# COMP6248-Reproducability-Challenge/selfsupervised-denoising

Measured on AMD Instinct MI355X. Metric: training patches/sec (64x64 gauss25 SSDN), higher is better.
Workload: dtype f16

## Files before the change

selfsupervised-denoising_amd/csrc/api.hip:

```cpp
#include "common.h"
#include <cstdarg>
#include <cstdio>
#include <cstdlib>

static thread_local char g_err[512] = "";
thread_local hipEvent_t g_ssdn_stop_event = nullptr;
thread_local bool g_ssdn_stop_used = false;
thread_local hipEvent_t g_ssdn_prof_start = nullptr, g_ssdn_prof_stop = nullptr;
thread_local bool g_ssdn_prof_used = false;

int ssdn_set_error(const char* fmt, ...) {
    va_list ap;
    va_start(ap, fmt);
    vsnprintf(g_err, sizeof(g_err), fmt, ap);
    va_end(ap);
    return -1;
}

#include <vector>
struct ProfSlot {
    bool on = false;
    std::vector<hipEvent_t> ev;
    size_t used = 0;
    double flops = 0.0, bytes = 0.0;
// ... 236 lines not shown
            armed = true;
        };
        switch (ops[i].type) {
            case SSDN_OP_PACK_INPUT: {
                const bool next_conv = i + 1 < n && ops[i + 1].type == SSDN_OP_CONV && ops[i + 1].args && (one_lane ? 0 : ops[i + 1].lane) == lane;
                if (next_conv && chain_merging_on() && conv_pack_fusable((const ssdn_pack_input_args*)p, (const ssdn_conv_args*)ops[i + 1].args)) {
                    rc = launch_conv_thin((const ssdn_conv_args*)ops[i + 1].args, (const ssdn_pack_input_args*)p, s);
                    ++i;
                } else rc = launch_pack_input((const ssdn_pack_input_args*)p, s);
                break;
            }
            case SSDN_OP_CONV: {
                const int m = chain_len(ops + i, n - i, one_lane);
                if (m < 0) return -1;
                const bool pair = m <= 1 && i + 1 < n && ops[i + 1].type == SSDN_OP_CONV && ops[i + 1].args && (one_lane ? 0 : ops[i + 1].lane) == lane &&
                                  chain_merging_on() && conv_pair_fusable((const ssdn_conv_args*)p, (const ssdn_conv_args*)ops[i + 1].args);
                arm(i + (m > 1 ? m : (pair ? 2 : 1)));
                if (m > 1) { rc = launch_chain(ops + i, m, one_lane, s); i += m - 1; }
                else if (pair) { rc = launch_gemm_dma_with_next((const ssdn_conv_args*)p, (const ssdn_conv_args*)ops[i + 1].args, s); ++i; }
                else rc = launch_conv((const ssdn_conv_args*)p, s);
                break;
            }
            case SSDN_OP_POOL_FWD: rc = launch_pool_fwd((const ssdn_pool_args*)p, s); break;
            case SSDN_OP_POOL_BWD: arm(i + 1); rc = launch_pool_bwd((const ssdn_pool_args*)p, s); break;
            case SSDN_OP_UPSUM_BWD: arm(i + 1); rc = launch_upsum_bwd((const ssdn_upsum_args*)p, s); break;
            case SSDN_OP_UNROT_FWD: rc = launch_unrot_fwd((const ssdn_unrot_args*)p, s); break;
            case SSDN_OP_UNROT_BWD: arm(i + 1); rc = launch_unrot_bwd((const ssdn_unrot_args*)p, s); break;
            case SSDN_OP_WGRAD: {
                static const bool no_merge = ssdn_tuning_env("SSDN_NO_WGRAD_MERGE") != nullptr;
                {
                    const ssdn_wgrad_args* mg[WGRAD_MEGA_MAX];
                    int mm = 0;
                    while (!no_merge && mm < WGRAD_MEGA_MAX && i + mm < n && ops[i + mm].type == SSDN_OP_WGRAD && ops[i + mm].args &&
                           (one_lane ? 0 : ops[i + mm].lane) == lane && wgrad_mega_ok((const ssdn_wgrad_args*)ops[i + mm].args) &&
                           ((const ssdn_wgrad_args*)ops[i + mm].args)->mega == ((const ssdn_wgrad_args*)p)->mega)
                        mg[mm] = (const ssdn_wgrad_args*)ops[i + mm].args, ++mm;
                    if (mm > 1) { arm(i + mm); rc = launch_wgrad_mega(mg, mm, s); i += mm - 1; break; }
                }
                const ssdn_wgrad_args* items[WGRAD_MULTI_MAX];
                int m = 0;
                while (!no_merge && m < WGRAD_MULTI_MAX && i + m < n && ops[i + m].type == SSDN_OP_WGRAD && ops[i + m].args &&
                       (one_lane ? 0 : ops[i + m].lane) == lane && wgrad_mergeable((const ssdn_wgrad_args*)ops[i + m].args))
                    items[m] = (const ssdn_wgrad_args*)ops[i + m].args, ++m;
                if (m > 1) { rc = launch_wgrad_multi(items, m, s); i += m - 1; }
                else rc = launch_wgrad((const ssdn_wgrad_args*)p, s);
                break;
            }
            case SSDN_OP_WREDUCE: {
                const ssdn_wreduce_args* items[WREDUCE_MULTI_MAX];
                int m = 0;
                while (m < WREDUCE_MULTI_MAX && i + m < n && ops[i + m].type == SSDN_OP_WREDUCE && ops[i + m].args &&
                       (one_lane ? 0 : ops[i + m].lane) == lane)
                    items[m] = (const ssdn_wreduce_args*)ops[i + m].args, ++m;
                arm_last(i + m);
                rc = m > 1 ? launch_wreduce_multi(items, m, s) : launch_wreduce((const ssdn_wreduce_args*)p, s);
                i += m - 1;
                break;
            }
            case SSDN_OP_WPACK: {
                const ssdn_wpack_args* items[WPACK_MULTI_MAX];
                int m = 0;
                while (m < WPACK_MULTI_MAX && i + m < n && ops[i + m].type == SSDN_OP_WPACK && ops[i + m].args &&
                       (one_lane ? 0 : ops[i + m].lane) == lane)
                    items[m] = (const ssdn_wpack_args*)ops[i + m].args, ++m;
                rc = m > 1 ? launch_wpack_multi(items, m, s) : launch_wpack((const ssdn_wpack_args*)p, s);
                i += m - 1;
                break;
            }
            case SSDN_OP_GRAD_PACK: {
                const bool next_conv = i + 1 < n && ops[i + 1].type == SSDN_OP_CONV && ops[i + 1].args && (one_lane ? 0 : ops[i + 1].lane) == lane;
                if (next_conv && chain_merging_on() && conv_gradpack_fusable((const ssdn_grad_pack_args*)p, (const ssdn_conv_args*)ops[i + 1].args)) {
                    arm(i + 2);
                    rc = launch_gradpack_dgrad((const ssdn_grad_pack_args*)p, (const ssdn_conv_args*)ops[i + 1].args, s);
                    ++i;
                } else { arm(i + 1); rc = launch_grad_pack((const ssdn_grad_pack_args*)p, s); }
                break;
            }
            case SSDN_OP_HEAD_SSDN: rc = launch_head((const ssdn_head_args*)p, s); break;
            case SSDN_OP_HEAD_FINAL: rc = launch_head_final((const ssdn_head_final_args*)p, s); break;
            case SSDN_OP_SPATIAL_MEAN: rc = launch_spatial_mean((const ssdn_spatial_mean_args*)p, s); break;
            case SSDN_OP_MSE: rc = launch_mse((const ssdn_mse_args*)p, 0, s); break;
            case SSDN_OP_MASK_MSE: rc = launch_mse((const ssdn_mse_args*)p, 1, s); break;
            case SSDN_OP_ADAM: {
                const ssdn_wpack_args* items[ADAM_PACK_MAX];
                int m = 0;
                while (m < ADAM_PACK_MAX && i + 1 + m < n && ops[i + 1 + m].type == SSDN_OP_WPACK && ops[i + 1 + m].args &&
                       (one_lane ? 0 : ops[i + 1 + m].lane) == lane)
                    items[m] = (const ssdn_wpack_args*)ops[i + 1 + m].args, ++m;
                const bool whole_run = !(i + 1 + m < n && ops[i + 1 + m].type == SSDN_OP_WPACK);
                if (m > 0 && whole_run && adam_pack_fusable((const ssdn_adam_args*)p, items, m)) {
                    rc = launch_adam_pack((const ssdn_adam_args*)p, items, m, s);
                    i += m;
                } else rc = launch_adam((const ssdn_adam_args*)p, s);
                break;
            }
            case SSDN_OP_METRICS: rc = launch_metrics((const ssdn_metrics_args*)p, s); break;
            case SSDN_OP_NOISE: rc = launch_noise((const ssdn_noise_args*)p, s); break;
            case SSDN_OP_INPUT_GRAD: arm(i + 1); rc = launch_input_grad((const ssdn_input_grad_args*)p, s); break;
            case SSDN_OP_HEAD_VJP: rc = launch_head_vjp((const ssdn_head_vjp_args*)p, s); break;
            case SSDN_OP_MSE_VJP: rc = launch_mse_vjp((const ssdn_mse_vjp_args*)p, s); break;
            case SSDN_OP_ACCUM: rc = launch_accum((const ssdn_accum_args*)p, s); break;
            case SSDN_OP_HEAD_POSTERIOR: rc = launch_head_posterior((const ssdn_head_posterior_args*)p, s); break;
            case SSDN_OP_SSIM: rc = launch_ssim((const ssdn_ssim_args*)p, s); break;
            case SSDN_OP_CALIBRATION: rc = launch_calibration((const ssdn_calibration_args*)p, s); break;
            case SSDN_OP_ZERO: {
                const ssdn_zero_args* z = (const ssdn_zero_args*)p;
// ... 74 lines not shown
```

selfsupervised-denoising_amd/csrc/common.h:

```cpp
#pragma once
#include <hip/hip_runtime.h>
#include <hip/hip_ext.h>
#include <stdint.h>
#include "../../include/ssdn_hip.h"
#include <cstdlib>

#if defined(SSDN_TUNING)
static inline const char* ssdn_tuning_env(const char* name) { return std::getenv(name); }
#else
static inline const char* ssdn_tuning_env(const char*) { return nullptr; }
#endif

typedef _Float16 h16;
typedef _Float16 half8 __attribute__((ext_vector_type(8)));
typedef _Float16 half4 __attribute__((ext_vector_type(4)));
typedef _Float16 half2v __attribute__((ext_vector_type(2)));
typedef __bf16 bf16x8 __attribute__((ext_vector_type(8)));
typedef unsigned short u16x8 __attribute__((ext_vector_type(8)));
typedef unsigned short u16x4 __attribute__((ext_vector_type(4)));
typedef float f32x16 __attribute__((ext_vector_type(16)));
typedef float f32x4 __attribute__((ext_vector_type(4)));

#define LRELU_SLOPE 0.1f

// ... 64 lines not shown
        } else if (g_ssdn_prof_start) {                                                                                          \
            hipExtLaunchKernelGGL(kernel, grid, block, lds, stream, g_ssdn_prof_start, g_ssdn_prof_stop, 0, __VA_ARGS__);        \
            g_ssdn_prof_start = nullptr;                                                                                         \
            g_ssdn_prof_used = true;                                                                                             \
        } else hipLaunchKernelGGL(kernel, grid, block, lds, stream, __VA_ARGS__);                                                \
    } while (0)

#define SSDN_MAX_DEVICES_ATTR 16
static inline int ssdn_current_device_slot() {
    int dev = 0;
    if (hipGetDevice(&dev) != hipSuccess || dev < 0) dev = 0;
    return dev % SSDN_MAX_DEVICES_ATTR;
}

void prof_begin(int kind, hipStream_t s);
void prof_end(int kind, hipStream_t s, double flops, double bytes);

int launch_conv(const ssdn_conv_args* a, hipStream_t s);
int launch_wgrad(const ssdn_wgrad_args* a, hipStream_t s);
bool wgrad_mergeable(const ssdn_wgrad_args* a);
int launch_wgrad_multi(const ssdn_wgrad_args* const* items, int n, hipStream_t s);
#define WGRAD_MEGA_MAX 64
int wgrad_mega_ok(const ssdn_wgrad_args* a);
int launch_wgrad_mega(const ssdn_wgrad_args* const* ops, int n, hipStream_t s);
int launch_pack_input(const ssdn_pack_input_args* a, hipStream_t s);
int launch_pool_fwd(const ssdn_pool_args* a, hipStream_t s);
int launch_pool_bwd(const ssdn_pool_args* a, hipStream_t s);
int launch_upsum_bwd(const ssdn_upsum_args* a, hipStream_t s);
int launch_unrot_fwd(const ssdn_unrot_args* a, hipStream_t s);
int launch_unrot_bwd(const ssdn_unrot_args* a, hipStream_t s);
int launch_wreduce(const ssdn_wreduce_args* a, hipStream_t s);
int launch_wpack(const ssdn_wpack_args* a, hipStream_t s);
#define WPACK_MULTI_MAX 24
int launch_wpack_multi(const ssdn_wpack_args* const* items, int n, hipStream_t s);
#define WREDUCE_MULTI_MAX 32
#define WGRAD_MULTI_MAX 32
int launch_wreduce_multi(const ssdn_wreduce_args* const* items, int n, hipStream_t s);
int launch_grad_pack(const ssdn_grad_pack_args* a, hipStream_t s);
int launch_head(const ssdn_head_args* a, hipStream_t s);
int launch_head_impulse(const ssdn_head_args* a, hipStream_t s);
int launch_head_final(const ssdn_head_final_args* a, hipStream_t s);
int launch_spatial_mean(const ssdn_spatial_mean_args* a, hipStream_t s);
int launch_mse(const ssdn_mse_args* a, int masked, hipStream_t s);
int launch_head_vjp(const ssdn_head_vjp_args* a, hipStream_t s);
int launch_head_vjp_impulse(const ssdn_head_vjp_args* a, hipStream_t s);
int launch_head_posterior(const ssdn_head_posterior_args* a, hipStream_t s);
int launch_ssim(const ssdn_ssim_args* a, hipStream_t s);
int launch_calibration(const ssdn_calibration_args* a, hipStream_t s);
int launch_mse_vjp(const ssdn_mse_vjp_args* a, hipStream_t s);
int launch_adam(const ssdn_adam_args* a, hipStream_t s);
#define ADAM_PACK_MAX 24
int adam_pack_fusable(const ssdn_adam_args* a, const ssdn_wpack_args* const* items, int n);
int launch_adam_pack(const ssdn_adam_args* a, const ssdn_wpack_args* const* items, int n, hipStream_t s);
int launch_metrics(const ssdn_metrics_args* a, hipStream_t s);
int launch_accum(const ssdn_accum_args* a, hipStream_t s);
int launch_noise(const ssdn_noise_args* a, hipStream_t s);
int launch_input_grad(const ssdn_input_grad_args* a, hipStream_t s);
int conv_lds_bytes(const ssdn_conv_args* a);
int conv_validate(const ssdn_conv_args* a);
int chain_len(const ssdn_op* ops, int n, bool any_lane);
int launch_chain(const ssdn_op* ops, int n, bool any_lane, hipStream_t s);
bool chain_merging_on();
bool conv_dma_eligible(const ssdn_conv_args* a, bool any_size);
int conv_dma_lds_bytes(int mt);
bool conv_signs(const ssdn_conv_args* a);
bool gemm_dma_signs(const ssdn_conv_args* a);
bool conv_dma_signs(const ssdn_conv_args* a);
bool conv_fuses_urot(const ssdn_conv_args* a);
bool conv_fuses_unrot(const ssdn_conv_args* a);
bool conv_fuses_upsum(const ssdn_conv_args* a);
bool conv_fuses_pool(const ssdn_conv_args* a);
int launch_conv_dma(const ssdn_conv_args* a, hipStream_t s);
bool conv_thin_eligible(const ssdn_conv_args* a);
bool conv_thin_fuses_pack(const ssdn_pack_input_args* pk, const ssdn_conv_args* a);
int launch_conv_thin(const ssdn_conv_args* a, const ssdn_pack_input_args* pk, hipStream_t s);
bool conv_pack_fusable(const ssdn_pack_input_args* pk, const ssdn_conv_args* a);
bool gradpack_dgrad_fusable(const ssdn_grad_pack_args* gp, const ssdn_conv_args* a);
int launch_gradpack_dgrad(const ssdn_grad_pack_args* gp, const ssdn_conv_args* a, hipStream_t s);
bool conv_gradpack_fusable(const ssdn_grad_pack_args* gp, const ssdn_conv_args* a);
bool gemm_dma_eligible(const ssdn_conv_args* a);
int gemm_dma_lds_bytes(const ssdn_conv_args* a);
int launch_gemm_dma(const ssdn_conv_args* a, hipStream_t s);
bool gemm_dma_fuses_next(const ssdn_conv_args* a, const ssdn_conv_args* b);
int launch_gemm_dma_with_next(const ssdn_conv_args* a, const ssdn_conv_args* b, hipStream_t s);
bool conv_pair_fusable(const ssdn_conv_args* a, const ssdn_conv_args* b);
extern "C" int ssdn_device_cus(void);
int wgrad_lds_bytes(const ssdn_wgrad_args* a);
```

selfsupervised-denoising_amd/csrc/elementwise.hip:

```cpp
#include "common.h"

#define EW_BLOCK 256
static inline int ew_grid(long long n) {
    long long g = (n + EW_BLOCK - 1) / EW_BLOCK;
    return (int)(g < 1 ? 1 : g);
}

__global__ void k_pack_input(ssdn_pack_input_args a) {
    const unsigned idx = blockIdx.x * blockDim.x + threadIdx.x;
    const int H = a.H, W = a.W;
    long long total = (long long)a.R * a.B * H * W;
    if (idx >= total) return;
    int j = idx % W;
    int i = (idx / W) % H;
    int nb = idx / (unsigned)(W * H);
    int r = nb / a.B, b = nb % a.B;
    int sy, sx;
    switch (r) {
        case 0: sy = i; sx = j; break;
        case 1: sy = j; sx = W - 1 - i; break;
        case 2: sy = H - 1 - i; sx = W - 1 - j; break;
        default: sy = H - 1 - j; sx = i; break;
    }
    h16* d = (h16*)a.dst.p + (long long)idx * a.dst.cs + a.dst.co;
    for (int c0 = 0; c0 < a.cpad; c0 += 8) {
        half8 v = zero_h8();
#pragma unroll
        for (int c = 0; c < 8; ++c)
            if (c0 + c < a.C) v[c] = (h16)a.src[(((long long)b * a.C + c0 + c) * H + sy) * W + sx];
        st_h8(d + c0, v);
    }
}
int launch_pack_input(const ssdn_pack_input_args* a, hipStream_t s) {
    if (a->R == 4 && a->H != a->W) return ssdn_set_error("pack_input: blind-spot rotation needs square images");
    long long n = (long long)a->R * a->B * a->H * a->W;
    if (n >= (1ll << 31)) return ssdn_set_error("pack_input: too many elements for 32-bit indexing");
    hipLaunchKernelGGL(k_pack_input, dim3(ew_grid(n)), dim3(EW_BLOCK), 0, s, *a);
    return 0;
}

__global__ void k_pool_fwd(ssdn_pool_args a) {
    const unsigned idx = blockIdx.x * blockDim.x + threadIdx.x;
    const int C8 = a.C >> 3, Ho = a.H >> 1, Wo = a.W >> 1;
    long long total = (long long)a.N * Ho * Wo * C8;
    if (idx >= total) return;
    int c = (idx % C8) * 8;
    const unsigned p = idx / C8;
    int j = p % Wo;
    int i = (p / Wo) % Ho;
    int n = p / (unsigned)(Wo * Ho);
    const h16* src = (const h16*)a.act.p + a.act.co + c;
    int r0 = a.shifted ? 2 * i - 1 : 2 * i;
    const bool padrow = a.shifted && r0 < 0;
    float m[8];
    unsigned win[8];
// ... 205 lines not shown
        int i, j;
        switch (r) {
            case 0: i = u; j = v; break;
            case 1: i = v; j = P - 1 - u; break;
            case 2: i = P - 1 - u; j = P - 1 - v; break;
            default: i = P - 1 - v; j = u; break;
        }
        u16x8 g = ld_b8((const unsigned short*)a.src.p + a.src.co + r * a.C + c + (((long long)b * P + i) * P + j) * a.src.cs);
        half8 mk = ld_h8((const h16*)a.mask.p + a.mask.co + c + (long long)p * a.mask.cs);
#pragma unroll
        for (int q = 0; q < 8; ++q) o[q] = f2bf(bf2f(g[q]) * lrelu_grad((float)mk[q]));
    }
    st_b8((unsigned short*)a.dst.p + a.dst.co + c + (long long)p * a.dst.cs, o);
}
int launch_unrot_bwd(const ssdn_unrot_args* a, hipStream_t s) {
    if (a->C & 7) return ssdn_set_error("unrot: C%%8 must be 0");
    long long n = (long long)4 * a->B * a->P * a->P * (a->C / 8);
    if (n >= (1ll << 31)) return ssdn_set_error("k_unrot_bwd: too many elements for 32-bit indexing");
    SSDN_LAUNCH(k_unrot_bwd, dim3(ew_grid(n)), dim3(EW_BLOCK), 0, s, *a);
    return 0;
}

__global__ void k_grad_pack(ssdn_grad_pack_args a) {
    const unsigned idx = blockIdx.x * blockDim.x + threadIdx.x;
    const unsigned HW = a.H * a.W;
    long long total = (long long)a.N * HW;
    if (idx == 0 && a.scale_out) {
        a.scale_out[0] = 1.f;
        a.scale_out[1] = 1.f;
    }
    if (idx >= total) return;
    int n = idx / HW;
    const unsigned pix = idx % HW;
    unsigned short* d = (unsigned short*)a.dst.p + a.dst.co + (long long)idx * a.dst.cs;
    for (int c0 = 0; c0 < a.cpad; c0 += 8) {
        u16x8 v = zero_b8();
#pragma unroll
        for (int c = 0; c < 8; ++c)
            if (c0 + c < a.C) v[c] = f2bf(a.g[((long long)n * a.C + c0 + c) * HW + pix]);
        st_b8(d + c0, v);
    }
}
int launch_grad_pack(const ssdn_grad_pack_args* a, hipStream_t s) {
    long long n = (long long)a->N * a->H * a->W;
    if (n >= (1ll << 31)) return ssdn_set_error("k_grad_pack: too many elements for 32-bit indexing");
    SSDN_LAUNCH(k_grad_pack, dim3(ew_grid(n)), dim3(EW_BLOCK), 0, s, *a);
    return 0;
}

static __device__ __forceinline__ int k_to_cin(int k, int c0, int c1_real) {
    if (k < c0) return k;
    int r = k - c0;
    return r < c1_real ? c0 + r : -1;
}
static __device__ __forceinline__ long long wpack_cm(int t, int m, int k, int rows, int K) {
    const int nfull = K / 48;
    const int c = k / 48 < nfull ? k / 48 : nfull;
    const int kk = k - c * 48, kcw = c < nfull ? 48 : 16;
    const int piece = (kk >> 3) ^ ((m >> 3) & 1);
    return (long long)t * rows * K + (long long)c * 48 * rows + (long long)m * kcw + piece * 8 + (kk & 7);
}
static __device__ __forceinline__ void wpack_element(const ssdn_wpack_args& a, long long idx) {
    long long nf = (long long)a.ntaps * a.Mpad_f * a.Ktot;
    long long nd = a.wd ? (long long)a.ntaps * a.Mpad_d * a.Kd : 0;
    if (idx < nf) {
        int k = idx % a.Ktot;
        int m = (idx / a.Ktot) % a.Mpad_f;
        int t = idx / ((long long)a.Ktot * a.Mpad_f);
        int ci = k_to_cin(k, a.c0, a.c1_real);
        float v = (m < a.M && ci >= 0) ? a.w[((long long)m * a.cin + ci) * a.ntaps + t] : 0.f;
        ((h16*)a.wf)[idx] = (h16)v;
        if (a.wfc) ((h16*)a.wfc)[wpack_cm(t, m, k, a.Mpad_f, a.Ktot)] = (h16)v;
    } else if (idx < nf + nd) {
        long long e = idx - nf;
        int m = e % a.Kd;
        int c = (e / a.Kd) % a.Mpad_d;
        int t = e / ((long long)a.Kd * a.Mpad_d);
        int ci = c < a.Ktot ? k_to_cin(c, a.c0, a.c1_real) : -1;
        float v = (m < a.M && ci >= 0) ? a.w[((long long)m * a.cin + ci) * a.ntaps + t] : 0.f;
        ((unsigned short*)a.wd)[e] = f2bf(v);
        if (a.wdc) ((unsigned short*)a.wdc)[wpack_cm(t, c, m, a.Mpad_d, a.Kd)] = f2bf(v);
    }
}
static inline long long wpack_count(const ssdn_wpack_args* a) {
    return (long long)a->ntaps * a->Mpad_f * a->Ktot + (a->wd ? (long long)a->ntaps * a->Mpad_d * a->Kd : 0);
}
__global__ void k_wpack(ssdn_wpack_args a) { wpack_element(a, (long long)blockIdx.x * blockDim.x + threadIdx.x); }
int launch_wpack(const ssdn_wpack_args* a, hipStream_t s) {
    hipLaunchKernelGGL(k_wpack, dim3(ew_grid(wpack_count(a))), dim3(EW_BLOCK), 0, s, *a);
    return 0;
}
struct WpackTable {
    ssdn_wpack_args e[WPACK_MULTI_MAX];
    int bstart[WPACK_MULTI_MAX + 1];
    int n;
};
__global__ void k_wpack_multi(WpackTable t) {
    int i = 0;
    while (i + 1 < t.n && (int)blockIdx.x >= t.bstart[i + 1]) ++i;
    wpack_element(t.e[i], (long long)(blockIdx.x - t.bstart[i]) * blockDim.x + threadIdx.x);
}
int launch_wpack_multi(const ssdn_wpack_args* const* items, int n, hipStream_t s) {
    if (n < 1 || n > WPACK_MULTI_MAX) return ssdn_set_error("wpack: bad batch size %d", n);
    WpackTable t;
    t.n = n;
    int b = 0;
    for (int i = 0; i < n; ++i) {
        t.e[i] = *items[i];
        t.bstart[i] = b;
        b += ew_grid(wpack_count(items[i]));
    }
    t.bstart[n] = b;
    if (b > 0) hipLaunchKernelGGL(k_wpack_multi, dim3(b), dim3(EW_BLOCK), 0, s, t);
// ... 119 lines not shown
    WrTable t1, t2;
    t1.n = t2.n = n;
    int b1 = 0, b2 = 0;
    for (int i = 0; i < n; ++i) {
        const ssdn_wreduce_args* a = items[i];
        const long long stride = (long long)a->ntaps * a->Mpad * a->Kpad;
        t1.e[i] = t2.e[i] = *a;
        t1.bstart[i] = b1;
        t2.bstart[i] = b2;
        if (a->nslabs > WR_GROUP) {
            t1.gx[i] = ew_grid(stride / 4);
            b1 += t1.gx[i] * ((a->nslabs + WR_GROUP - 1) / WR_GROUP);
            t2.step[i] = WR_GROUP;
        } else {
            t1.gx[i] = 0;
            t2.step[i] = 1;
        }
        t1.step[i] = t2.step[i];
        t2.gx[i] = t1.gx[i];
        if (a->Kpad & 3) return ssdn_set_error("wreduce: Kpad must be a multiple of 4");
        b2 += ew_grid(stride / 4 + a->M);
    }
    t1.bstart[n] = b1;
    t2.bstart[n] = b2;
    if (b1 > 0) hipLaunchKernelGGL(k_wreduce_partial_multi, dim3(b1), dim3(EW_BLOCK), 0, s, t1);
    if (b2 > 0) SSDN_LAUNCH(k_wreduce_multi, dim3(b2), dim3(EW_BLOCK), 0, s, t2);
    return 0;
}

int launch_wreduce(const ssdn_wreduce_args* a, hipStream_t s) {
    long long stride = (long long)a->ntaps * a->Mpad * a->Kpad;
    int step = 1;
    if (a->nslabs > WR_GROUP) {
        int groups = (a->nslabs + WR_GROUP - 1) / WR_GROUP;
        hipLaunchKernelGGL(k_wreduce_partial, dim3(ew_grid(stride / 4), groups), dim3(EW_BLOCK), 0, s, (float*)a->slab, stride, a->nslabs);
        step = WR_GROUP;
    }
    if (a->Kpad & 3) return ssdn_set_error("wreduce: Kpad must be a multiple of 4");
    long long n = stride / 4 + a->M;
    SSDN_LAUNCH(k_wreduce, dim3(ew_grid(n)), dim3(EW_BLOCK), 0, s, *a, step);
    return 0;
}

__global__ void k_accum(ssdn_accum_args a) {
    const long long i = (long long)blockIdx.x * blockDim.x + threadIdx.x;
    if (i < a.n) a.dst[i] = __fadd_rn(a.dst[i], a.src[i]);
}
int launch_accum(const ssdn_accum_args* a, hipStream_t s) {
    if (!a->dst || !a->src || a->n < 0) return ssdn_set_error("accum: dst and src must be given, n >= 0");
    if (a->n > 0) hipLaunchKernelGGL(k_accum, dim3(ew_grid(a->n)), dim3(EW_BLOCK), 0, s, *a);
    return 0;
}

struct AdamIn { float g, m, v, p; };
static __device__ __forceinline__ AdamIn adam_load(const ssdn_adam_args& a, long long i) { return AdamIn{a.g[i], a.m[i], a.v[i], a.p[i]}; }
static __device__ __forceinline__ float adam_apply(const ssdn_adam_args& a, long long i, const AdamIn& q, float inv_bc2s, float step) {
    const float g = q.g * a.gscale;
    const float m = __fmaf_rn(a.b1, q.m, __fmul_rn(1.f - a.b1, g));
    const float v = __fmaf_rn(a.b2, q.v, __fmul_rn(__fmul_rn(1.f - a.b2, g), g));
    a.m[i] = m;
    a.v[i] = v;
    const float den = __fmaf_rn(sqrtf(v), inv_bc2s, a.eps);
    const float pn = __fsub_rn(q.p, __fdiv_rn(__fmul_rn(step, m), den));
    a.p[i] = pn;
    return pn;
}
static __device__ __forceinline__ float adam_elem(const ssdn_adam_args& a, long long i, float inv_bc2s, float step) {
    return adam_apply(a, i, adam_load(a, i), inv_bc2s, step);
}
__global__ void k_adam(ssdn_adam_args a) {
    long long i = (long long)blockIdx.x * blockDim.x + threadIdx.x;
    long long stride = (long long)gridDim.x * blockDim.x;
    float inv_bc2s = 1.f / sqrtf(a.bc2);
    float step = a.lr / a.bc1;
    for (; i < a.n; i += stride) adam_elem(a, i, inv_bc2s, step);
}
#define AP_TM 8
#define AP_TK 48
struct AdamPackTable {
    ssdn_adam_args a;
    ssdn_wpack_args e[ADAM_PACK_MAX];
    long long w_off[ADAM_PACK_MAX];
    int bstart[ADAM_PACK_MAX + 1];
    int tiles_k[ADAM_PACK_MAX];
    long long gap_start[ADAM_PACK_MAX + 2];
    long long gap_end[ADAM_PACK_MAX + 2];
    int gap_bstart[ADAM_PACK_MAX + 3];
    int n, ngaps;
};
template <int NT>
static __device__ __forceinline__ void adam_pack_tile(const AdamPackTable& t, int j, int tile, float* lds, float inv_bc2s, float step) {
    const ssdn_adam_args& a = t.a;
    const ssdn_wpack_args& w = t.e[j];
    const int tk = t.tiles_k[j];
    const int mo0 = (tile / tk) * AP_TM, k0 = (tile % tk) * AP_TK;
    const int tid = threadIdx.x;
    constexpr int TOTAL = AP_TM * AP_TK * NT, NIT = (TOTAL + EW_BLOCK - 1) / EW_BLOCK, BATCH = NIT < 7 ? NIT : 7;
#pragma unroll
    for (int it0 = 0; it0 < NIT; it0 += BATCH) {
        AdamIn q[BATCH];
        long long idx[BATCH];
        bool ok[BATCH];
#pragma unroll
        for (int u = 0; u < BATCH; ++u) {
            const int e = tid + (it0 + u) * EW_BLOCK;
            const int mo = e / (AP_TK * NT), r = e - mo * (AP_TK * NT);
            const int kk = r / NT, tp = r - kk * NT;
            ok[u] = it0 + u < NIT && e < TOTAL && mo0 + mo < w.M && k0 + kk < w.cin;
            idx[u] = ok[u] ? t.w_off[j] + ((long long)(mo0 + mo) * w.cin + k0 + kk) * NT + tp : t.w_off[j];
            q[u] = adam_load(a, idx[u]);
        }
#pragma unroll
        for (int u = 0; u < BATCH; ++u) {
            const int e = tid + (it0 + u) * EW_BLOCK;
            if (it0 + u >= NIT || e >= TOTAL) continue;
            const int mo = e / (AP_TK * NT), r = e - mo * (AP_TK * NT);
            const int kk = r / NT, tp = r - kk * NT;
            lds[(tp * AP_TM + mo) * (AP_TK + 1) + kk] = ok[u] ? adam_apply(a, idx[u], q[u], inv_bc2s, step) : 0.f;
        }
    }
    __syncthreads();
    for (int e = tid; e < NT * AP_TM * AP_TK; e += EW_BLOCK) {
        const int tp = e / (AP_TM * AP_TK), r = e - tp * (AP_TM * AP_TK);
        const int mo = r / AP_TK, kk = r - mo * AP_TK;
        const int m = mo0 + mo, k = k0 + kk;
        if (m >= w.M || k >= w.cin) continue;
        const float pn = lds[(tp * AP_TM + mo) * (AP_TK + 1) + kk];
        ((h16*)w.wf)[((long long)tp * w.Mpad_f + m) * w.Ktot + k] = (h16)pn;
        if (w.wfc) ((h16*)w.wfc)[wpack_cm(tp, m, k, w.Mpad_f, w.Ktot)] = (h16)pn;
    }
    if (w.wd) {
        for (int e = tid; e < NT * AP_TK * AP_TM; e += EW_BLOCK) {
            const int tp = e / (AP_TK * AP_TM), r = e - tp * (AP_TK * AP_TM);
            const int kk = r / AP_TM, mo = r - kk * AP_TM;
            const int m = mo0 + mo, k = k0 + kk;
            if (m >= w.M || k >= w.cin || k >= w.Mpad_d || m >= w.Kd) continue;
            const float pn = lds[(tp * AP_TM + mo) * (AP_TK + 1) + kk];
            ((unsigned short*)w.wd)[((long long)tp * w.Mpad_d + k) * w.Kd + m] = f2bf(pn);
            if (w.wdc) ((unsigned short*)w.wdc)[wpack_cm(tp, k, m, w.Mpad_d, w.Kd)] = f2bf(pn);
        }
    }
}
__global__ void k_adam_pack(AdamPackTable t) {
    __shared__ float lds[9 * AP_TM * (AP_TK + 1)];
    const ssdn_adam_args& a = t.a;
    const float inv_bc2s = 1.f / sqrtf(a.bc2);
    const float step = a.lr / a.bc1;
    const int b = blockIdx.x;
    if (b < t.bstart[t.n]) {
        int j = 0;
        while (j + 1 < t.n && b >= t.bstart[j + 1]) ++j;
        if (t.e[j].ntaps == 9) adam_pack_tile<9>(t, j, b - t.bstart[j], lds, inv_bc2s, step);
        else adam_pack_tile<1>(t, j, b - t.bstart[j], lds, inv_bc2s, step);
    } else {
        int g = 0;
        while (g + 1 < t.ngaps && b >= t.gap_bstart[g + 1]) ++g;
        const long long first = t.gap_start[g] + (long long)(b - t.gap_bstart[g]) * (EW_BLOCK * 4) + threadIdx.x;
#pragma unroll
        for (int u = 0; u < 4; ++u) {
            const long long i = first + u * EW_BLOCK;
            if (i < t.gap_end[g]) adam_elem(a, i, inv_bc2s, step);
        }
    }
}
int adam_pack_fusable(const ssdn_adam_args* a, const ssdn_wpack_args* const* items, int n) {
    if (n < 1 || n > ADAM_PACK_MAX) return 0;
    long long prev = -1;
    for (int i = 0; i < n; ++i) {
        const ssdn_wpack_args* w = items[i];
        const long long off = w->w - a->p;
        if (w->w < a->p || off + (long long)w->M * w->cin * w->ntaps > a->n || off <= prev) return 0;
        if (w->c0 + w->c1_real != w->cin || (w->ntaps != 1 && w->ntaps != 9)) return 0;
        prev = off;
    }
    return 1;
}
int launch_adam_pack(const ssdn_adam_args* a, const ssdn_wpack_args* const* items, int n, hipStream_t s) {
    AdamPackTable t;
    t.a = *a;
    t.n = n;
    int blocks = 0, ng = 0;
    long long pos = 0;
    auto gap = [&](long long start, long long end) {
        if (end <= start) return;
        t.gap_start[ng] = start; t.gap_end[ng] = end;
        ++ng;
    };
    for (int i = 0; i < n; ++i) {
        t.e[i] = *items[i];
        t.w_off[i] = items[i]->w - a->p;
        t.bstart[i] = blocks;
        t.tiles_k[i] = (items[i]->cin + AP_TK - 1) / AP_TK;
        blocks += ((items[i]->M + AP_TM - 1) / AP_TM) * t.tiles_k[i];
        gap(pos, t.w_off[i]);
// ... 174 lines not shown
```

Before: 20570.

## Fuse weight-gradient slab reduction with Adam update and weight packing into one kernel

Adds a tail-fused kernel that reduces the per-slab weight-gradient partials straight into LDS, feeds the reduced gradient into the Adam update, and writes the packed f16/bf16 weight layouts in the same block. This replaces the separate wreduce and adam+pack launches, removing a launch and a round trip of the gradient through global memory. A host-side plan with a load-balanced block list (splitting heavy 3x3 tiles) is built once and cached in device memory, keyed on the argument contents. The cost is more LDS per block, eligibility checks on each call, and a large new scheduling path that only runs when the layout constraints hold.

Result: faster. 20780, median of 6 (+1.0%).

```diff
diff --git a/selfsupervised-denoising_amd/csrc/adam_pack.h b/selfsupervised-denoising_amd/csrc/adam_pack.h
--- /dev/null
+++ b/selfsupervised-denoising_amd/csrc/adam_pack.h
@@ -0,0 +1,93 @@
+#pragma once
+#include "common.h"
+
+#ifndef EW_BLOCK
+#define EW_BLOCK 256
+#endif
+
+static __device__ __forceinline__ long long wpack_cm(int t, int m, int k, int rows, int K) {
+    const int nfull = K / 48;
+    const int c = k / 48 < nfull ? k / 48 : nfull;
+    const int kk = k - c * 48, kcw = c < nfull ? 48 : 16;
+    const int piece = (kk >> 3) ^ ((m >> 3) & 1);
+    return (long long)t * rows * K + (long long)c * 48 * rows + (long long)m * kcw + piece * 8 + (kk & 7);
+}
+
+struct AdamIn { float g, m, v, p; };
+static __device__ __forceinline__ AdamIn adam_load(const ssdn_adam_args& a, long long i) { return AdamIn{a.g[i], a.m[i], a.v[i], a.p[i]}; }
+static __device__ __forceinline__ float adam_apply(const ssdn_adam_args& a, long long i, const AdamIn& q, float inv_bc2s, float step) {
+    const float g = q.g * a.gscale;
+    const float m = __fmaf_rn(a.b1, q.m, __fmul_rn(1.f - a.b1, g));
+    const float v = __fmaf_rn(a.b2, q.v, __fmul_rn(__fmul_rn(1.f - a.b2, g), g));
+    a.m[i] = m;
+    a.v[i] = v;
+    const float den = __fmaf_rn(sqrtf(v), inv_bc2s, a.eps);
+    const float pn = __fsub_rn(q.p, __fdiv_rn(__fmul_rn(step, m), den));
+    a.p[i] = pn;
+    return pn;
+}
+static __device__ __forceinline__ float adam_elem(const ssdn_adam_args& a, long long i, float inv_bc2s, float step) {
+    return adam_apply(a, i, adam_load(a, i), inv_bc2s, step);
+}
+
+#define AP_TM 8
+#define AP_TK 48
+template <int TK>
+static __device__ __forceinline__ int ap_slot(int tp, int mo, int kk) { return (tp * AP_TM + mo) * (TK + 1) + kk; }
+struct ApGradFromMemory {
+    const float* g;
+    __device__ __forceinline__ float operator()(long long idx, bool, int) const { return g[idx]; }
+};
+template <int NT, int TK, class GSRC>
+static __device__ __forceinline__ void adam_pack_update(const ssdn_adam_args& a, const ssdn_wpack_args& w, long long w_off, int mo0, int k0,
+                                                        float* lds, float inv_bc2s, float step, const GSRC& gsrc) {
+    const int tid = threadIdx.x;
+    constexpr int TOTAL = AP_TM * TK * NT, NIT = (TOTAL + EW_BLOCK - 1) / EW_BLOCK, BATCH = NIT < 7 ? NIT : 7;
+#pragma unroll
+    for (int it0 = 0; it0 < NIT; it0 += BATCH) {
+        AdamIn q[BATCH];
+        long long idx[BATCH];
+        bool ok[BATCH];
+#pragma unroll
+        for (int u = 0; u < BATCH; ++u) {
+            const int e = tid + (it0 + u) * EW_BLOCK;
+            const int mo = e / (TK * NT), r = e - mo * (TK * NT);
+            const int kk = r / NT, tp = r - kk * NT;
+            ok[u] = it0 + u < NIT && e < TOTAL && mo0 + mo < w.M && k0 + kk < w.cin;
+            idx[u] = ok[u] ? w_off + ((long long)(mo0 + mo) * w.cin + k0 + kk) * NT + tp : w_off;
+            q[u] = AdamIn{gsrc(idx[u], ok[u], ap_slot<TK>(tp, mo, kk)), a.m[idx[u]], a.v[idx[u]], a.p[idx[u]]};
+        }
+#pragma unroll
+        for (int u = 0; u < BATCH; ++u) {
+            const int e = tid + (it0 + u) * EW_BLOCK;
+            if (it0 + u >= NIT || e >= TOTAL) continue;
+            const int mo = e / (TK * NT), r = e - mo * (TK * NT);
+            const int kk = r / NT, tp = r - kk * NT;
+            lds[ap_slot<TK>(tp, mo, kk)] = ok[u] ? adam_apply(a, idx[u], q[u], inv_bc2s, step) : 0.f;
+        }
+    }
+}
+template <int NT, int TK>
+static __device__ __forceinline__ void adam_pack_store(const ssdn_wpack_args& w, int mo0, int k0, const float* lds) {
+    const int tid = threadIdx.x;
+    for (int e = tid; e < NT * AP_TM * TK; e += EW_BLOCK) {
+        const int tp = e / (AP_TM * TK), r = e - tp * (AP_TM * TK);
+        const int mo = r / TK, kk = r - mo * TK;
+        const int m = mo0 + mo, k = k0 + kk;
+        if (m >= w.M || k >= w.cin) continue;
+        const float pn = lds[ap_slot<TK>(tp, mo, kk)];
+        ((h16*)w.wf)[((long long)tp * w.Mpad_f + m) * w.Ktot + k] = (h16)pn;
+        if (w.wfc) ((h16*)w.wfc)[wpack_cm(tp, m, k, w.Mpad_f, w.Ktot)] = (h16)pn;
+    }
+    if (w.wd) {
+        for (int e = tid; e < NT * TK * AP_TM; e += EW_BLOCK) {
+            const int tp = e / (TK * AP_TM), r = e - tp * (TK * AP_TM);
+            const int kk = r / AP_TM, mo = r - kk * AP_TM;
+            const int m = mo0 + mo, k = k0 + kk;
+            if (m >= w.M || k >= w.cin || k >= w.Mpad_d || m >= w.Kd) continue;
+            const float pn = lds[ap_slot<TK>(tp, mo, kk)];
+            ((unsigned short*)w.wd)[((long long)tp * w.Mpad_d + k) * w.Kd + m] = f2bf(pn);
+            if (w.wdc) ((unsigned short*)w.wdc)[wpack_cm(tp, k, m, w.Mpad_d, w.Kd)] = f2bf(pn);
+        }
+    }
+}
diff --git a/selfsupervised-denoising_amd/csrc/api.hip b/selfsupervised-denoising_amd/csrc/api.hip
--- a/selfsupervised-denoising_amd/csrc/api.hip
+++ b/selfsupervised-denoising_amd/csrc/api.hip
@@ -312,6 +312,28 @@
                 while (m < WREDUCE_MULTI_MAX && i + m < n && ops[i + m].type == SSDN_OP_WREDUCE && ops[i + m].args &&
                        (one_lane ? 0 : ops[i + m].lane) == lane)
                     items[m] = (const ssdn_wreduce_args*)ops[i + m].args, ++m;
+                static const bool no_tail = ssdn_tuning_env("SSDN_NO_TAIL_FUSE") != nullptr;
+                const int ia = i + m;
+                const bool more_red = ia < n && ops[ia].type == SSDN_OP_WREDUCE && (one_lane ? 0 : ops[ia].lane) == lane;
+                if (!no_tail && !more_red && ia < n && ops[ia].type == SSDN_OP_ADAM && ops[ia].args && (one_lane ? 0 : ops[ia].lane) == lane) {
+                    const ssdn_wpack_args* packs[ADAM_PACK_MAX];
+                    int mp = 0;
+                    while (mp < ADAM_PACK_MAX && ia + 1 + mp < n && ops[ia + 1 + mp].type == SSDN_OP_WPACK && ops[ia + 1 + mp].args &&
+                           (one_lane ? 0 : ops[ia + 1 + mp].lane) == lane)
+                        packs[mp] = (const ssdn_wpack_args*)ops[ia + 1 + mp].args, ++mp;
+                    const bool whole_run = !(ia + 1 + mp < n && ops[ia + 1 + mp].type == SSDN_OP_WPACK);
+                    const ssdn_adam_args* ad = (const ssdn_adam_args*)ops[ia].args;
+                    if (mp > 0 && whole_run && adam_pack_fusable(ad, packs, mp)) {
+                        const int ok = tail_fused_ok(items, m, ad, packs, mp);
+                        if (ok < 0) return -1;
+                        if (ok) {
+                            arm_last(ia + 1 + mp);
+                            rc = launch_tail_fused(items, m, ad, packs, mp, s);
+                            i = ia + mp;
+                            break;
+                        }
+                    }
+                }
                 arm_last(i + m);
                 rc = m > 1 ? launch_wreduce_multi(items, m, s) : launch_wreduce((const ssdn_wreduce_args*)p, s);
                 i += m - 1;
diff --git a/selfsupervised-denoising_amd/csrc/common.h b/selfsupervised-denoising_amd/csrc/common.h
--- a/selfsupervised-denoising_amd/csrc/common.h
+++ b/selfsupervised-denoising_amd/csrc/common.h
@@ -140,6 +140,8 @@
 #define ADAM_PACK_MAX 24
 int adam_pack_fusable(const ssdn_adam_args* a, const ssdn_wpack_args* const* items, int n);
 int launch_adam_pack(const ssdn_adam_args* a, const ssdn_wpack_args* const* items, int n, hipStream_t s);
+int tail_fused_ok(const ssdn_wreduce_args* const* wr, int nw, const ssdn_adam_args* a, const ssdn_wpack_args* const* wp, int np);
+int launch_tail_fused(const ssdn_wreduce_args* const* wr, int nw, const ssdn_adam_args* a, const ssdn_wpack_args* const* wp, int np, hipStream_t s);
 int launch_metrics(const ssdn_metrics_args* a, hipStream_t s);
 int launch_accum(const ssdn_accum_args* a, hipStream_t s);
 int launch_noise(const ssdn_noise_args* a, hipStream_t s);
diff --git a/selfsupervised-denoising_amd/csrc/elementwise.hip b/selfsupervised-denoising_amd/csrc/elementwise.hip
--- a/selfsupervised-denoising_amd/csrc/elementwise.hip
+++ b/selfsupervised-denoising_amd/csrc/elementwise.hip
@@ -1,6 +1,6 @@
 #include "common.h"
-
-#define EW_BLOCK 256
+#include "adam_pack.h"
+
 static inline int ew_grid(long long n) {
     long long g = (n + EW_BLOCK - 1) / EW_BLOCK;
     return (int)(g < 1 ? 1 : g);
@@ -312,13 +312,6 @@
     if (k < c0) return k;
     int r = k - c0;
     return r < c1_real ? c0 + r : -1;
-}
-static __device__ __forceinline__ long long wpack_cm(int t, int m, int k, int rows, int K) {
-    const int nfull = K / 48;
-    const int c = k / 48 < nfull ? k / 48 : nfull;
-    const int kk = k - c * 48, kcw = c < nfull ? 48 : 16;
-    const int piece = (kk >> 3) ^ ((m >> 3) & 1);
-    return (long long)t * rows * K + (long long)c * 48 * rows + (long long)m * kcw + piece * 8 + (kk & 7);
 }
 static __device__ __forceinline__ void wpack_element(const ssdn_wpack_args& a, long long idx) {
     long long nf = (long long)a.ntaps * a.Mpad_f * a.Ktot;
@@ -544,22 +537,6 @@
     return 0;
 }
 
-struct AdamIn { float g, m, v, p; };
-static __device__ __forceinline__ AdamIn adam_load(const ssdn_adam_args& a, long long i) { return AdamIn{a.g[i], a.m[i], a.v[i], a.p[i]}; }
-static __device__ __forceinline__ float adam_apply(const ssdn_adam_args& a, long long i, const AdamIn& q, float inv_bc2s, float step) {
-    const float g = q.g * a.gscale;
-    const float m = __fmaf_rn(a.b1, q.m, __fmul_rn(1.f - a.b1, g));
-    const float v = __fmaf_rn(a.b2, q.v, __fmul_rn(__fmul_rn(1.f - a.b2, g), g));
-    a.m[i] = m;
-    a.v[i] = v;
-    const float den = __fmaf_rn(sqrtf(v), inv_bc2s, a.eps);
-    const float pn = __fsub_rn(q.p, __fdiv_rn(__fmul_rn(step, m), den));
-    a.p[i] = pn;
-    return pn;
-}
-static __device__ __forceinline__ float adam_elem(const ssdn_adam_args& a, long long i, float inv_bc2s, float step) {
-    return adam_apply(a, i, adam_load(a, i), inv_bc2s, step);
-}
 __global__ void k_adam(ssdn_adam_args a) {
     long long i = (long long)blockIdx.x * blockDim.x + threadIdx.x;
     long long stride = (long long)gridDim.x * blockDim.x;
@@ -567,8 +544,6 @@
     float step = a.lr / a.bc1;
     for (; i < a.n; i += stride) adam_elem(a, i, inv_bc2s, step);
 }
-#define AP_TM 8
-#define AP_TK 48
 struct AdamPackTable {
     ssdn_adam_args a;
     ssdn_wpack_args e[ADAM_PACK_MAX];
@@ -582,56 +557,12 @@
 };
 template <int NT>
 static __device__ __forceinline__ void adam_pack_tile(const AdamPackTable& t, int j, int tile, float* lds, float inv_bc2s, float step) {
-    const ssdn_adam_args& a = t.a;
     const ssdn_wpack_args& w = t.e[j];
     const int tk = t.tiles_k[j];
     const int mo0 = (tile / tk) * AP_TM, k0 = (tile % tk) * AP_TK;
-    const int tid = threadIdx.x;
-    constexpr int TOTAL = AP_TM * AP_TK * NT, NIT = (TOTAL + EW_BLOCK - 1) / EW_BLOCK, BATCH = NIT < 7 ? NIT : 7;
-#pragma unroll
-    for (int it0 = 0; it0 < NIT; it0 += BATCH) {
-        AdamIn q[BATCH];
-        long long idx[BATCH];
-        bool ok[BATCH];
-#pragma unroll
-        for (int u = 0; u < BATCH; ++u) {
-            const int e = tid + (it0 + u) * EW_BLOCK;
-            const int mo = e / (AP_TK * NT), r = e - mo * (AP_TK * NT);
-            const int kk = r / NT, tp = r - kk * NT;
-            ok[u] = it0 + u < NIT && e < TOTAL && mo0 + mo < w.M && k0 + kk < w.cin;
-            idx[u] = ok[u] ? t.w_off[j] + ((long long)(mo0 + mo) * w.cin + k0 + kk) * NT + tp : t.w_off[j];
-            q[u] = adam_load(a, idx[u]);
-        }
-#pragma unroll
-        for (int u = 0; u < BATCH; ++u) {
-            const int e = tid + (it0 + u) * EW_BLOCK;
-            if (it0 + u >= NIT || e >= TOTAL) continue;
-            const int mo = e / (AP_TK * NT), r = e - mo * (AP_TK * NT);
-            const int kk = r / NT, tp = r - kk * NT;
-            lds[(tp * AP_TM + mo) * (AP_TK + 1) + kk] = ok[u] ? adam_apply(a, idx[u], q[u], inv_bc2s, step) : 0.f;
-        }
-    }
+    adam_pack_update<NT, AP_TK>(t.a, w, t.w_off[j], mo0, k0, lds, inv_bc2s, step, ApGradFromMemory{t.a.g});
     __syncthreads();
-    for (int e = tid; e < NT * AP_TM * AP_TK; e += EW_BLOCK) {
-        const int tp = e / (AP_TM * AP_TK), r = e - tp * (AP_TM * AP_TK);
-        const int mo = r / AP_TK, kk = r - mo * AP_TK;
-        const int m = mo0 + mo, k = k0 + kk;
-        if (m >= w.M || k >= w.cin) continue;
-        const float pn = lds[(tp * AP_TM + mo) * (AP_TK + 1) + kk];
-        ((h16*)w.wf)[((long long)tp * w.Mpad_f + m) * w.Ktot + k] = (h16)pn;
-        if (w.wfc) ((h16*)w.wfc)[wpack_cm(tp, m, k, w.Mpad_f, w.Ktot)] = (h16)pn;
-    }
-    if (w.wd) {
-        for (int e = tid; e < NT * AP_TK * AP_TM; e += EW_BLOCK) {
-            const int tp = e / (AP_TK * AP_TM), r = e - tp * (AP_TK * AP_TM);
-            const int kk = r / AP_TM, mo = r - kk * AP_TM;
-            const int m = mo0 + mo, k = k0 + kk;
-            if (m >= w.M || k >= w.cin || k >= w.Mpad_d || m >= w.Kd) continue;
-            const float pn = lds[(tp * AP_TM + mo) * (AP_TK + 1) + kk];
-            ((unsigned short*)w.wd)[((long long)tp * w.Mpad_d + k) * w.Kd + m] = f2bf(pn);
-            if (w.wdc) ((unsigned short*)w.wdc)[wpack_cm(tp, k, m, w.Mpad_d, w.Kd)] = f2bf(pn);
-        }
-    }
+    adam_pack_store<NT, AP_TK>(w, mo0, k0, lds);
 }
 __global__ void k_adam_pack(AdamPackTable t) {
     __shared__ float lds[9 * AP_TM * (AP_TK + 1)];
diff --git a/selfsupervised-denoising_amd/csrc/tail_fused.hip b/selfsupervised-denoising_amd/csrc/tail_fused.hip
--- /dev/null
+++ b/selfsupervised-denoising_amd/csrc/tail_fused.hip
@@ -0,0 +1,333 @@
+#include "adam_pack.h"
+#include <cstring>
+#include <mutex>
+#include <vector>
+#include <algorithm>
+
+#define TF_GROUP 32
+#define TF_MAX_GROUPS 8
+#define TF_TKQ (AP_TK / 4)
+#ifndef TF_SPLIT_BYTES
+#define TF_SPLIT_BYTES (256 << 10)
+#endif
+#ifndef TF_DEPTH
+#define TF_DEPTH 8
+#endif
+#define TF_STRETCH (EW_BLOCK * 4)
+
+struct TfSeg { long long start; int len, entry; };
+struct TfBlock {
+    int layer;
+    int tile;
+    int entry;
+    int sub;
+};
+struct TfTable {
+    ssdn_wpack_args e[ADAM_PACK_MAX];
+    ssdn_wreduce_args r[WREDUCE_MULTI_MAX];
+    TfSeg seg[WREDUCE_MULTI_MAX];
+    long long w_off[ADAM_PACK_MAX];
+    long long gap_start[ADAM_PACK_MAX + 2];
+    long long gap_end[ADAM_PACK_MAX + 2];
+    int tiles_k[ADAM_PACK_MAX];
+    int n, nent, ngaps, nseg, nblocks, pad[3];
+};
+typedef const __attribute__((address_space(4))) TfTable* TfTableC;
+typedef const __attribute__((address_space(4))) TfBlock* TfBlockC;
+
+static __device__ __forceinline__ float4 tf_chain(const float4* p, long long st4, int s0, int s1) {
+    float4 acc = make_float4(0.f, 0.f, 0.f, 0.f);
+    for (int s = s0; s < s1; s += TF_DEPTH) {
+        float4 v[TF_DEPTH];
+#pragma unroll
+        for (int u = 0; u < TF_DEPTH; ++u)
+            if (s + u < s1) v[u] = p[(long long)(s + u) * st4];
+#pragma unroll
+        for (int u = 0; u < TF_DEPTH; ++u)
+            if (s + u < s1) { acc.x += v[u].x; acc.y += v[u].y; acc.z += v[u].z; acc.w += v[u].w; }
+    }
+    return acc;
+}
+struct TfGradFromSlabs {
+    float* gw;
+    const float* psum;
+    int groups, gstride;
+    float inv;
+    __device__ __forceinline__ float operator()(long long idx, bool ok, int slot) const {
+        if (!ok) return 0.f;
+        float sum = psum[slot];
+        if (groups > 1) {
+            sum = 0.f + sum;
+            for (int g = 1; g < groups; ++g) sum += psum[g * gstride + slot];
+        }
+        const float gr = __fmul_rn(sum, inv);
+        gw[idx] = gr;
+        return gr;
+    }
+};
+template <int NT, int TK>
+static __device__ __forceinline__ void tf_tile(const TfTable& t, const ssdn_adam_args& a, int j, int ent, int mo0, int k0, float* lds,
+                                               float inv_bc2s, float step) {
+    const ssdn_wpack_args& w = t.e[j];
+    if (ent < 0) adam_pack_update<NT, TK>(a, w, t.w_off[j], mo0, k0, lds, inv_bc2s, step, ApGradFromMemory{a.g});
+    else {
+        const ssdn_wreduce_args& r = t.r[ent];
+        constexpr int K4 = TK / 4, F = NT * AP_TM * K4, SLOTS = NT * AP_TM * (TK + 1);
+        const int groups = (r.nslabs + TF_GROUP - 1) / TF_GROUP;
+        const int ml0 = mo0 - r.m_off, kl0 = k0 - r.c_off;
+        const long long st4 = ((long long)r.ntaps * r.Mpad * r.Kpad) >> 2;
+        for (int item = threadIdx.x; item < groups * F; item += EW_BLOCK) {
+            const int g = item / F, f = item - g * F;
+            const int row = f / K4, k4 = f - row * K4;
+            const int tp = row / AP_TM, mo = row - tp * AP_TM;
+            const int ml = ml0 + mo, kl = kl0 + 4 * k4;
+            if (ml >= r.M || kl >= r.cin) continue;
+            const float4* p = reinterpret_cast<const float4*>(r.slab + ((long long)tp * r.Mpad + ml) * r.Kpad + kl);
+            const int s0 = g * TF_GROUP, s1 = s0 + TF_GROUP < r.nslabs ? s0 + TF_GROUP : r.nslabs;
+            const float4 acc = tf_chain(p, st4, s0, s1);
+            float* d = lds + g * SLOTS + ap_slot<TK>(tp, mo, 4 * k4);
+            d[0] = acc.x; d[1] = acc.y; d[2] = acc.z; d[3] = acc.w;
+        }
+        __syncthreads();
+        const TfGradFromSlabs gsrc{const_cast<float*>(a.g), lds, groups, SLOTS, r.inv_scale ? *r.inv_scale : 1.f};
+        adam_pack_update<NT, TK>(a, w, t.w_off[j], mo0, k0, lds, inv_bc2s, step, gsrc);
+    }
+    __syncthreads();
+    adam_pack_store<NT, TK>(w, mo0, k0, lds);
+}
+
+__global__ __launch_bounds__(EW_BLOCK) void k_tail_fused(const TfTable* __restrict__ tab, const TfBlock* __restrict__ blocks, ssdn_adam_args a) {
+    extern __shared__ __attribute__((aligned(16))) float tf_lds[];
+    const TfTable& t = *(const TfTable*)(TfTableC)(unsigned long long)tab;
+    const TfBlockC bp = (TfBlockC)(unsigned long long)(blocks + blockIdx.x);
+    const int layer = bp->layer, tile = bp->tile, ent = bp->entry, sub = bp->sub;
+    const float inv_bc2s = 1.f / sqrtf(a.bc2);
+    const float step = a.lr / a.bc1;
+    if (layer >= 0) {
+        const int tk = t.tiles_k[layer];
+        const int mo0 = (tile / tk) * AP_TM, k0 = (tile % tk) * AP_TK;
+        if (t.e[layer].ntaps == 9) {
+            if (sub < 0) tf_tile<9, AP_TK>(t, a, layer, ent, mo0, k0, tf_lds, inv_bc2s, step);
+            else tf_tile<9, TF_TKQ>(t, a, layer, ent, mo0, k0 + sub * TF_TKQ, tf_lds, inv_bc2s, step);
+        } else tf_tile<1, AP_TK>(t, a, layer, ent, mo0, k0, tf_lds, inv_bc2s, step);
+    } else {
+        const int gp = -1 - layer;
+        const long long first = t.gap_start[gp] + (long long)tile * TF_STRETCH + threadIdx.x;
+#pragma unroll
+        for (int u = 0; u < 4; ++u) {
+            const long long i = first + u * EW_BLOCK;
+            if (i >= t.gap_end[gp]) continue;
+            int e = -1, m = 0;
+            for (int q = 0; q < sub; ++q) {
+                const long long d = i - t.seg[ent + q].start;
+                if (d >= 0 && d < t.seg[ent + q].len) { e = t.seg[ent + q].entry; m = (int)d; }
+            }
+            if (e < 0) { adam_elem(a, i, inv_bc2s, step); continue; }
+            const ssdn_wreduce_args& r = t.r[e];
+            float acc = 0.f;
+            int s = 0;
+            for (; s + 16 <= r.nslabs; s += 16) {
+                float v[16];
+#pragma unroll
+                for (int x = 0; x < 16; ++x) v[x] = r.bslab[(long long)(s + x) * r.Mpad + m];
+#pragma unroll
+                for (int x = 0; x < 16; ++x) acc += v[x];
+            }
+            for (; s < r.nslabs; ++s) acc += r.bslab[(long long)s * r.Mpad + m];
+            const float gr = __fmul_rn(acc, r.inv_scale ? *r.inv_scale : 1.f);
+            const_cast<float*>(a.g)[i] = gr;
+            adam_apply(a, i, AdamIn{gr, a.m[i], a.v[i], a.p[i]}, inv_bc2s, step);
+        }
+    }
+}
+
+namespace {
+struct TfPlan {
+    TfTable t;
+    std::vector<TfBlock> blocks;
+    size_t lds;
+};
+struct TfCache {
+    std::vector<char> key;
+    char* dev;
+    int device, nblocks;
+    size_t lds;
+};
+std::vector<TfCache> g_tf_cache;
+std::mutex g_tf_mutex;
+}
+
+static bool tail_fusable(const ssdn_wreduce_args* const* wr, int nw, const ssdn_adam_args* a, const ssdn_wpack_args* const* wp, int np, TfPlan* out) {
+    if (nw < 1 || nw > WREDUCE_MULTI_MAX || np < 1 || np > ADAM_PACK_MAX || !a->g || !a->p) return false;
+    TfTable& t = out->t;
+    memset(&t, 0, sizeof(t));
+    t.n = np; t.nent = nw;
+    long long pos = 0;
+    int ng = 0;
+    auto gap = [&](long long start, long long end) {
+        if (end <= start) return;
+        t.gap_start[ng] = start; t.gap_end[ng] = end;
+        ++ng;
+    };
+    for (int i = 0; i < np; ++i) {
+        t.e[i] = *wp[i];
+        t.w_off[i] = wp[i]->w - a->p;
+        t.tiles_k[i] = (wp[i]->cin + AP_TK - 1) / AP_TK;
+        gap(pos, t.w_off[i]);
+        pos = t.w_off[i] + (long long)wp[i]->M * wp[i]->cin * wp[i]->ntaps;
+    }
+    gap(pos, a->n);
+    t.ngaps = ng;
+    int layer_of[WREDUCE_MULTI_MAX];
+    for (int i = 0; i < nw; ++i) {
+        const ssdn_wreduce_args* r = wr[i];
+        if (r->accumulate || r->tapblock || (r->Kpad & 3) || r->nslabs < 1 || r->nslabs > TF_GROUP * TF_MAX_GROUPS) return false;
+        if (!r->slab || !r->gw || r->M < 1 || r->cin < 1 || r->M > r->Mpad || r->cin > r->Kpad || r->m_off < 0 || r->c_off < 0) return false;
+        int j = -1;
+        for (int l = 0; l < np; ++l)
+            if (r->gw == a->g + t.w_off[l]) j = l;
+        if (j < 0) return false;
+        const ssdn_wpack_args* w = wp[j];
+        if (r->ntaps != w->ntaps || r->cin_full != w->cin) return false;
+        const int m1 = r->m_off + r->M, c1 = r->c_off + r->cin;
+        if (m1 > w->M || c1 > w->cin) return false;
+        if (r->m_off % AP_TM || (m1 % AP_TM && m1 != w->M) || r->c_off % AP_TK || (c1 % AP_TK && c1 != w->cin)) return false;
+        for (int q = 0; q < i; ++q)
+            if (layer_of[q] == j && r->m_off < wr[q]->m_off + wr[q]->M && wr[q]->m_off < m1 && r->c_off < wr[q]->c_off + wr[q]->cin && wr[q]->c_off < c1)
+                return false;
+        layer_of[i] = j;
+        t.r[i] = *r;
+        if (r->gb) {
+            if (!r->bslab) return false;
+            const long long start = (r->gb - a->g) + r->m_off;
+            bool inside = false;
+            for (int g = 0; g < ng; ++g) inside = inside || (start >= t.gap_start[g] && start + r->M <= t.gap_end[g]);
+            if (r->gb < a->g || !inside) return false;
+            for (int q = 0; q < t.nseg; ++q)
+                if (start < t.seg[q].start + t.seg[q].len && t.seg[q].start < start + r->M) return false;
+            t.seg[t.nseg++] = TfSeg{start, r->M, i};
+        }
+    }
+    std::stable_sort(t.seg, t.seg + t.nseg, [](const TfSeg& x, const TfSeg& y) { return x.start < y.start; });
+    struct Unit { long long cost; TfBlock b; };
+    std::vector<Unit> heavy, rest;
+    size_t lds = 0;
+    for (int j = 0; j < np; ++j) {
+        const ssdn_wpack_args* w = wp[j];
+        const int tm = (w->M + AP_TM - 1) / AP_TM, tk = t.tiles_k[j];
+        for (int tile = 0; tile < tm * tk; ++tile) {
+            const int mo0 = (tile / tk) * AP_TM, k0 = (tile % tk) * AP_TK;
+            int ent = -1;
+            for (int i = 0; i < nw; ++i)
+                if (layer_of[i] == j && mo0 >= wr[i]->m_off && mo0 < wr[i]->m_off + wr[i]->M && k0 >= wr[i]->c_off && k0 < wr[i]->c_off + wr[i]->cin) ent = i;
+            const int kw = std::min(AP_TK, w->cin - k0);
+            const long long elems = (long long)w->ntaps * AP_TM * kw;
+            const long long bytes = elems * 16 + (ent >= 0 ? elems * 4 * wr[ent]->nslabs : 0);
+            const int groups = ent >= 0 ? (wr[ent]->nslabs + TF_GROUP - 1) / TF_GROUP : 1;
+            if (ent >= 0 && w->ntaps == 9 && (long long)9 * AP_TM * AP_TK * 4 * wr[ent]->nslabs > TF_SPLIT_BYTES) {
+                for (int sub = 0; sub * TF_TKQ < kw; ++sub) heavy.push_back({bytes / ((kw + TF_TKQ - 1) / TF_TKQ), TfBlock{j, tile, ent, sub}});
+                lds = std::max(lds, (size_t)groups * 9 * AP_TM * (TF_TKQ + 1) * 4);
+            } else {
+                rest.push_back({bytes, TfBlock{j, tile, ent, -1}});
+                lds = std::max(lds, (size_t)groups * w->ntaps * AP_TM * (AP_TK + 1) * 4);
+            }
+        }
+    }
+    for (int g = 0; g < ng; ++g) {
+        const int nb = (int)((t.gap_end[g] - t.gap_start[g] + TF_STRETCH - 1) / TF_STRETCH);
+        for (int b = 0; b < nb; ++b) {
+            const long long lo = t.gap_start[g] + (long long)b * TF_STRETCH, hi = std::min(lo + TF_STRETCH, t.gap_end[g]);
+            int first = -1, cnt = 0;
+            long long bytes = (hi - lo) * 16;
+            for (int q = 0; q < t.nseg; ++q)
+                if (t.seg[q].start < hi && lo < t.seg[q].start + t.seg[q].len) {
+                    if (first < 0) first = q;
+                    cnt = q - first + 1;
+                    bytes += (long long)t.seg[q].len * 4 * wr[t.seg[q].entry]->nslabs;
+                }
+            rest.push_back({bytes, TfBlock{-1 - g, b, first < 0 ? 0 : first, cnt}});
+        }
+    }
+    std::stable_sort(heavy.begin(), heavy.end(), [](const Unit& x, const Unit& y) { return x.cost > y.cost; });
+    std::vector<TfBlock>& blocks = out->blocks;
+    blocks.clear();
+    size_t h = 0;
+    while (h < heavy.size()) {
+        size_t tiles_first[9];
+        int nt = 0;
+        size_t q = h;
+        while (q < heavy.size() && nt < 8) {
+            tiles_first[nt++] = q;
+            const TfBlock& b0 = heavy[q].b;
+            while (q < heavy.size() && heavy[q].b.layer == b0.layer && heavy[q].b.tile == b0.tile) ++q;
+        }
+        tiles_first[nt] = q;
+        for (int sub = 0; sub < 4; ++sub)
+            for (int k = 0; k < nt; ++k)
+                if (tiles_first[k] + sub < tiles_first[k + 1]) blocks.push_back(heavy[tiles_first[k] + sub].b);
+        h = q;
+    }
+    std::stable_sort(rest.begin(), rest.end(), [](const Unit& x, const Unit& y) { return x.cost > y.cost; });
+    for (const Unit& u : rest) blocks.push_back(u.b);
+    t.nblocks = (int)blocks.size();
+    out->lds = lds;
+    return t.nblocks > 0 && lds <= 64 * 1024;
+}
+
+static int tf_lookup(const ssdn_wreduce_args* const* wr, int nw, const ssdn_adam_args* a, const ssdn_wpack_args* const* wp, int np,
+                     char** dtab, int* nblocks, size_t* lds) {
+    *dtab = nullptr;
+    if (nw < 1 || nw > WREDUCE_MULTI_MAX || np < 1 || np > ADAM_PACK_MAX) return 0;
+    struct { const void *p, *g, *m, *v; long long n; int nw, np; } head = {a->p, a->g, a->m, a->v, (long long)a->n, nw, np};
+    std::vector<char> key(sizeof(head) + (size_t)nw * sizeof(ssdn_wreduce_args) + (size_t)np * sizeof(ssdn_wpack_args));
+    memcpy(key.data(), &head, sizeof(head));
+    for (int i = 0; i < nw; ++i) memcpy(key.data() + sizeof(head) + (size_t)i * sizeof(ssdn_wreduce_args), wr[i], sizeof(ssdn_wreduce_args));
+    for (int i = 0; i < np; ++i)
+        memcpy(key.data() + sizeof(head) + (size_t)nw * sizeof(ssdn_wreduce_args) + (size_t)i * sizeof(ssdn_wpack_args), wp[i], sizeof(ssdn_wpack_args));
+    int dev = 0;
+    SSDN_CHECK_HIP(hipGetDevice(&dev));
+    std::lock_guard<std::mutex> lock(g_tf_mutex);
+    const TfCache* hit = nullptr;
+    for (const TfCache& c : g_tf_cache)
+        if (c.device == dev && c.key.size() == key.size() && !memcmp(c.key.data(), key.data(), key.size())) { hit = &c; break; }
+    if (!hit) {
+        if (g_tf_cache.size() >= 64) {
+            SSDN_CHECK_HIP(hipDeviceSynchronize());
+            if (g_tf_cache.front().dev) SSDN_CHECK_HIP(hipFree(g_tf_cache.front().dev));
+            g_tf_cache.erase(g_tf_cache.begin());
+        }
+        TfPlan plan;
+        TfCache c{key, nullptr, dev, 0, 0};
+        if (tail_fusable(wr, nw, a, wp, np, &plan)) {
+            const size_t bytes = sizeof(TfTable) + sizeof(TfBlock) * plan.blocks.size();
+            std::vector<char> host(bytes);
+            memcpy(host.data(), &plan.t, sizeof(TfTable));
+            memcpy(host.data() + sizeof(TfTable), plan.blocks.data(), sizeof(TfBlock) * plan.blocks.size());
+            SSDN_CHECK_HIP(hipMalloc((void**)&c.dev, bytes));
+            SSDN_CHECK_HIP(hipMemcpy(c.dev, host.data(), bytes, hipMemcpyHostToDevice));
+            c.nblocks = plan.t.nblocks;
+            c.lds = plan.lds;
+        }
+        g_tf_cache.push_back(c);
+        hit = &g_tf_cache.back();
+    }
+    *dtab = hit->dev; *nblocks = hit->nblocks; *lds = hit->lds;
+    return 0;
+}
+int tail_fused_ok(const ssdn_wreduce_args* const* wr, int nw, const ssdn_adam_args* a, const ssdn_wpack_args* const* wp, int np) {
+    char* dtab;
+    int nblocks;
+    size_t lds;
+    const int rc = tf_lookup(wr, nw, a, wp, np, &dtab, &nblocks, &lds);
+    return rc ? rc : (dtab ? 1 : 0);
+}
+int launch_tail_fused(const ssdn_wreduce_args* const* wr, int nw, const ssdn_adam_args* a, const ssdn_wpack_args* const* wp, int np, hipStream_t s) {
+    char* dtab;
+    int nblocks;
+    size_t lds;
+    const int rc = tf_lookup(wr, nw, a, wp, np, &dtab, &nblocks, &lds);
+    if (rc) return rc;
+    if (!dtab) return ssdn_set_error("tail_fused: the run is not fusable");
+    SSDN_LAUNCH(k_tail_fused, dim3((unsigned)nblocks), dim3(EW_BLOCK), lds, s, (const TfTable*)dtab, (const TfBlock*)(dtab + sizeof(TfTable)), *a);
+    return 0;
+}
```
